# zju3dv/instant-nvr

Measured on AMD Instinct MI355X. Metric: ray-samples/sec, higher is better.
Workload: dtype f32

## Files before the change

include/invr.h:

```cpp
#ifndef INVR_H
#define INVR_H

#include <stddef.h>
#include <stdint.h>

#ifdef __cplusplus
extern "C" {
#endif

#define INVR_NUM_PARTS 5
#define INVR_MAX_LEVELS 16
#define INVR_MAX_LINEAR 4
#define INVR_NUM_JOINTS 24

typedef struct InvrGrid {
    const float* dense;
    const float* hash;
    const float* bounds;
    int32_t n_levels;
    int32_t n_features;
    int32_t start_hash;
    int32_t separate_dense;
    int64_t table_len;
    int32_t res[INVR_MAX_LEVELS];
    float cell[INVR_MAX_LEVELS];
    int64_t dense_off[INVR_MAX_LEVELS];
    int32_t sum;
    int32_t sum_over_features;
    int32_t include_input;
    const float* row_sums;
} InvrGrid;

typedef struct InvrMlp {
    const float* weight[INVR_MAX_LINEAR];
    const float* bias[INVR_MAX_LINEAR];
    int32_t dims[INVR_MAX_LINEAR + 1];
    int32_t n_linear;
} InvrMlp;

typedef struct InvrPart {
    InvrGrid grid;
    InvrMlp occ;
    InvrMlp rgb;
    const float* rgb_latent;
    int32_t latent_dim;
    int32_t num_latent_code;
} InvrPart;

typedef struct InvrModel {
    InvrPart part[INVR_NUM_PARTS];
    InvrGrid deform_grid;
    InvrMlp deform_mlp;
// ... 288 lines not shown
```

instant-nvr_amd/_abi.py:

```python
import ctypes as C
import os

import torch

from . import params
from .config import NUM_PARTS, PART_NAMES

HERE = os.path.dirname(os.path.abspath(__file__))
LIB_PATH = os.environ.get('INVR_LIB_PATH') or os.path.join(HERE, 'libinvr.so')

MAX_LEVELS, MAX_LINEAR, STATS_LEN = 16, 4, 16
_f32p, _f64p, _i32p, _i64p, _u8p = C.POINTER(C.c_float), C.POINTER(C.c_double), C.POINTER(C.c_int32), C.POINTER(C.c_int64), C.POINTER(C.c_uint8)


class InvrGrid(C.Structure):
    _fields_ = [('dense', C.c_void_p), ('hash', C.c_void_p), ('bounds', C.c_void_p),
                ('n_levels', C.c_int32), ('n_features', C.c_int32), ('start_hash', C.c_int32),
                ('separate_dense', C.c_int32), ('table_len', C.c_int64),
                ('res', C.c_int32 * MAX_LEVELS), ('cell', C.c_float * MAX_LEVELS),
                ('dense_off', C.c_int64 * MAX_LEVELS),
                ('sum', C.c_int32), ('sum_over_features', C.c_int32), ('include_input', C.c_int32),
                ('row_sums', C.c_void_p)]


class InvrMlpBwdOut(C.Structure):
    _fields_ = [('g_emb', C.c_void_p), ('gz', C.c_void_p), ('a', C.c_void_p), ('n_pad', C.c_int64), ('g_latent', C.c_void_p)]


class InvrDeformBwdOut(C.Structure):
    _fields_ = [(k, C.c_void_p) for k in ('uvt', 'gfeat', 'gz1', 'gz2', 'gz3', 'a0', 'a1', 'a2')]


class InvrAdamTensor(C.Structure):
    _fields_ = [('param', C.c_void_p), ('grad', C.c_void_p), ('exp_avg', C.c_void_p), ('exp_avg_sq', C.c_void_p),
                ('numel', C.c_int64), ('lr', C.c_float), ('weight_decay', C.c_float), ('bc1', C.c_float), ('bc2_sqrt', C.c_float),
                ('active', C.c_void_p), ('grad_shift', C.c_int32), ('step', C.c_int32)]


class InvrPartGrads(C.Structure):
    _fields_ = [('row_grad', C.c_void_p), ('occ_w', C.c_void_p * 4), ('occ_b', C.c_void_p * 4), ('rgb_w', C.c_void_p * 4),
                ('rgb_b', C.c_void_p * 4), ('rgb_latent', C.c_void_p)]


class InvrTrainGrads(C.Structure):
    _fields_ = [('part', InvrPartGrads * NUM_PARTS), ('deform_dense', C.c_void_p), ('deform_hash', C.c_void_p),
# ... 130 lines not shown
    return {
        'invr_grid_points': (C.c_int, [f3, f3, i3, i64, i64, vp, vp]),
        'invr_mesh_workspace_bytes': (size, [i3]),
        'invr_mesh_workspace_layout': (C.c_int, [i3, C.POINTER(InvrMeshLayout)]),
        'invr_mesh_count': (C.c_int, [vp, i3, f32, vp, size, vp, vp]),
        'invr_mesh_emit': (C.c_int, [vp, i3, f3, f3, f32, vp, size, vp, i64, vp, i64, vp, vp]),
    }


def _signatures_batch():
    i32, vp = C.c_int32, C.c_void_p
    return {
        'invr_patch_batch': (C.c_int, [vp, vp, i32, i32, i32, i32, i32, i32, _f32p, _f64p, _f64p, _f64p, _f32p, vp, vp, vp, vp, vp, vp, vp, vp, vp]),
    }


def _signatures_sample():
    i32, vp = C.c_int32, C.c_void_p
    return {
        'invr_ray_batch': (C.c_int, [vp, vp, vp, vp, i32, i32, vp, i32, _f64p, _f64p, _f64p, _f64p, _f32p, vp, vp, vp, vp, vp, vp, vp]),
    }


SIGNATURES = _signatures()
SIGNATURES_PERCEPTUAL = _signatures_perceptual()
SIGNATURES_MESH = _signatures_mesh()
SIGNATURES_BATCH = _signatures_batch()
SIGNATURES_SAMPLE = _signatures_sample()
EXPORTS = list(SIGNATURES)
ABI_VERSION = 2
BWD_HEAD, BWD_DEFORMER, BWD_ALL = 1, 64, 127
EVAL_RESULT_BYTES = 64
NUM_STAGES = 14
STAGE_NAMES = ['cull', 'knn', 'warp'] + ['encode_%d' % p for p in range(5)] + ['mlp_%d' % p for p in range(5)] + ['composite']

_lib = None


def lib():
    global _lib
    if _lib is None:
        if not os.path.exists(LIB_PATH):
            raise RuntimeError('libinvr.so is not built (%s); run `python -c "import __graft_entry__ as g; g.build()"`. '
                               'There is no CPU fallback for the render path.' % LIB_PATH)
        L = C.CDLL(LIB_PATH)
        for name, (restype, argtypes) in (list(SIGNATURES.items()) + list(SIGNATURES_PERCEPTUAL.items()) + list(SIGNATURES_MESH.items())
                                          + list(SIGNATURES_BATCH.items()) + list(SIGNATURES_SAMPLE.items())):
            fn = getattr(L, name)
            fn.restype, fn.argtypes = restype, list(argtypes)
        if L.invr_version() != ABI_VERSION:
            raise RuntimeError('libinvr.so speaks ABI version %d, this binding %d (include/invr.h INVR_ABI_VERSION): rebuild the library '
                               '(python -m invr.build)' % (L.invr_version(), ABI_VERSION))
        for i, t in enumerate((InvrGrid, InvrMlp, InvrPart, InvrModel, InvrScene, InvrWsLayout, InvrMlpBwdOut, InvrAdamTensor, InvrTrainGrads,
                               InvrDeformBwdOut)):
            if L.invr_sizeof(i) != C.sizeof(t):
                raise RuntimeError('libinvr ABI mismatch: struct %s is %d bytes in the library, %d in the binding'
                                   % (t.__name__, L.invr_sizeof(i), C.sizeof(t)))
        _lib = L
    return _lib


def profile_enable(on):
    lib().invr_profile_enable(int(bool(on)))


def profile_read():
    ms = (C.c_float * NUM_STAGES)()
    n = C.c_int32(0)
    check(lib().invr_profile_read(ms, C.byref(n)))
    return {STAGE_NAMES[i]: float(ms[i]) for i in range(NUM_STAGES)}, int(n.value)
# ... 185 lines not shown
```

instant-nvr_amd/build.py:

```python
import os
import subprocess
import sys
from concurrent.futures import ThreadPoolExecutor

HERE = os.path.dirname(os.path.abspath(__file__))
CSRC = os.path.join(HERE, 'csrc')
OUT = os.path.join(HERE, 'libinvr.so')
SOURCES = ['invr_abi.hip', 'k_cull.hip', 'k_knn.hip', 'k_warp.hip', 'k_encode.hip', 'k_mlp.hip', 'k_composite.hip', 'k_rays.hip', 'k_prep.hip', 'k_optim.hip', 'k_mlp_bwd.hip', 'k_train.hip', 'k_metrics.hip', 'k_perceptual.hip', 'k_mesh.hip', 'k_batch.hip', 'k_sample.hip']
INCLUDE = os.path.join(HERE, '..', 'include')


def headers():
    return ([os.path.join(CSRC, h) for h in sorted(os.listdir(CSRC)) if h.endswith('.h')]
            + [os.path.join(INCLUDE, h) for h in ('invr.h', 'invr_perceptual.h', 'invr_mesh.h', 'invr_batch.h', 'invr_sample.h')])


FLAGS = ['--offload-arch=gfx950', '-O3', '-std=c++17', '-fPIC', '-ffp-contract=off', '-fno-slp-vectorize', '-Wall', '-Wno-unused-function']


def hipcc():
    for c in (os.environ.get('HIPCC'), '/opt/rocm/bin/hipcc', 'hipcc'):
        if c and (os.path.sep not in c or os.path.exists(c)):
            return c
    raise RuntimeError('hipcc not found')


def _stale(target, deps):
    if not os.path.exists(target):
        return True
    t = os.path.getmtime(target)
    return any(os.path.getmtime(d) > t for d in deps)


def build(force=False, verbose=True):
    cc = hipcc()
    objdir = os.path.join(HERE, 'build')
    os.makedirs(objdir, exist_ok=True)
# ... 38 lines not shown
```

instant-nvr_amd/config.py:

```python
import copy

PART_NAMES = ['body', 'leg', 'head', 'larm', 'rarm']
NUM_PARTS = 5
PART_BW_MAP = {
    'body': [14, 13, 9, 6, 3, 0],
    'leg': [1, 2, 4, 5, 7, 8, 10, 11],
    'head': [12, 15],
    'larm': [16, 18, 20, 22],
    'rarm': [17, 19, 21, 23],
}
HASH_PRIMES = (1, 19349663, 83492791)


class Node(dict):

    def __getattr__(self, k):
        try:
            return self[k]
        except KeyError:
            raise AttributeError(k)

    def __setattr__(self, k, v):
        self[k] = v

# ... 25 lines not shown
    'tpose_viewdir': True,
    'use_pair_reg': True,
    'use_reg_distortion': True,
    'random_bg': False,
    'latent_code_dim': 8,
    'geo_feature_dim': 16,
    'num_train_frame': 100,
    'num_latent_code': 100,
    'knn_k': 4,
    'use_knn': True,
    'part_deform': False,
    'use_amp': False,
    'use_batch_bounds': True,
    'bbox_overlap': 0.2,
    'pair_loss_weight': 10.0,
    'reg_dist_weight': 0.1,
    'resd_loss_weight': 0.1,
    'train_fused_loss': True,
    'fused_perceptual': True,
    'train_fused': True,
    'train_hip_mlp': True,
    'voxel_size': [0.005, 0.005, 0.005],
    'eval_row_sums': True,
    'use_lpips': False, 'use_ssim': False, 'use_fourier': False, 'use_tv_image': False, 'vgg19_weights': None,
    'patch_size': 64, 'sample_focus': '',
    'N_rand': 1024, 'body_sample_ratio': 0.5, 'face_sample_ratio': 0.0, 'patch_sampling': False,
    'prune_using_geo': False, 'train_with_coord': False, 'sample_using_mse': False,
    'network': {'occ': {'d_hidden': 64, 'n_layers': 1}},
    'viewdir_embedder': {'kwargs': {'res': 4, 'input_dims': 3}},
    'tpose_deformer': {'embedder': {'kwargs': dict(
        n_levels=8, n_features_per_level=2, log2_hashmap_size=14, base_resolution=4, b=1.38,
        sum=False, sum_over_features=True, separate_dense=True, use_batch_bounds=False,
        include_input=True)}},
    'partnet': {
        'body': _part(20, 16, [[-1, -1.2, -0.34], [0.8, 0.7, 0.5]], 2),
        'leg': _part(20, 2, [[-1, -1.2, -0.34], [0.8, -0.3, 0.5]], 1),
        'head': _part(18, 2, [[-0.3, 0.3, -0.3], [0.3, 0.7, 0.3]], 2),
        'larm': _part(15, 2, [[0.2, 0, -0.2], [0.9, 0.35, 0.2]], 1),
        'rarm': _part(15, 2, [[-0.9, 0, -0.2], [-0.2, 0.35, 0.2]], 1),
    },
}


def make_cfg(**overrides):
    d = copy.deepcopy(DEFAULTS)
    table_log2 = overrides.pop('table_log2', None)
# ... 82 lines not shown
```

instant-nvr_amd/csrc/common.h:

```cpp
#pragma once
#include <hip/hip_runtime.h>
#include <stdint.h>
#include "../../include/invr.h"

#define INVR_WAVE 64
#if defined(__HIP_DEVICE_COMPILE__) && !defined(__gfx950__)
#error "libinvr is written for gfx950 (MI355X) only: build with --offload-arch=gfx950"
#endif
#define HASH_P1 19349663ull
#define HASH_P2 83492791ull

void invr_set_error(const char* fmt, ...);
#define INVR_CHECK(cond, ...)                \
    do {                                     \
        if (!(cond)) {                       \
            invr_set_error(__VA_ARGS__);     \
            return 1;                        \
        }                                    \
    } while (0)
#define INVR_HIP(call)                                                              \
    do {                                                                            \
        hipError_t e_ = (call);                                                     \
        if (e_ != hipSuccess) {                                                     \
            invr_set_error("%s failed: %s", #call, hipGetErrorString(e_));          \
// ... 12 lines not shown

static inline int64_t cdiv(int64_t a, int64_t b) { return (a + b - 1) / b; }
static inline size_t align_up(size_t x, size_t a) { return (x + a - 1) / a * a; }

struct GridDev {
    const float* dense;
    const float* hash;
    const float* bounds;
    int32_t L, F, start_hash, separate_dense;
    int64_t T;
    double inv_T;
    int32_t mod_k, mod32;
    uint32_t mod_c;
    int32_t xdelta;
    int32_t mod1r;
    int32_t mod24;
    int32_t res[INVR_MAX_LEVELS];
    float cell[INVR_MAX_LEVELS];
    float rcell[INVR_MAX_LEVELS];
    int64_t dense_off[INVR_MAX_LEVELS];
    int32_t sum, sum_over_features, include_input;
    const float* row_sums;
    int64_t dense_rows;
};

struct VolDev {
    const float* data;
    const float* bounds;
    int32_t dx, dy, dz, c;
};

struct SceneDev {
    const float* R;
    const float* Th;
    const float* A;
    const float* big_A;
    VolDev pbw;
    VolDev tuv;
    const float* part_pts;
    const float* part_pbw;
    const int64_t* lengths2;
    int32_t M;
    const float* frame_dim;
    const int64_t* latent_index;
    float thresh;
    int32_t tpose_viewdir;
// ... 208 lines not shown
}

int launch_grid_encode_generic(const GridDev& g, const float* xyz, int64_t n, float* out, hipStream_t st);
int launch_grid_encode_bwd_generic(const GridDev& g, const float* xyz, const float* gout, int64_t n, float* g_dense,
                                   float* g_hash, float* g_xyz, hipStream_t st, const int32_t* count = nullptr);
int launch_part_encode_bwd_lists(const GridDev& g, const float* x_soa, const float* gout_soa, float* gx_soa, int64_t stride,
                                 int64_t n_max, const int32_t* count, float* rowgrad, hipStream_t st);
int launch_composite_bwd(const float* raw, const float* g_rgb, const float* g_acc, const float* g_w, int64_t n_rays, int S, float eps,
                         float* g_raw, hipStream_t st);
int launch_sample_volume(const VolDev& v, int c0, int nc, const float* pts, int64_t n, float* out, hipStream_t st);
int launch_knn_blend_dense(const SceneDev& s, const float* pose_pts, int64_t n, float* bw, float* dist, int32_t* nn, float* d2,
                           float* w, hipStream_t st);
int launch_warp_deform_dense(const SceneDev& s, const GridDev& dg, const MlpDev& dm, const float* pose_pts,
                             const float* pose_dirs, const float* bw, const uint8_t* flag, int64_t n,
                             float* tpose, float* tdirs, float* resd, hipStream_t st);
int launch_deform_points(const SceneDev& s, const GridDev& dg, const MlpDev& dm, const float* pts, int64_t n, float* out, hipStream_t st);
int launch_distortion(const float* weights, const float* z, int64_t n_rays, int S, float* out, hipStream_t st);
int launch_generate_rays(const double* kinv, const double* r, const double* t, const double* o, const float* bounds,
                         int H, int W, float* ray_d, float* near, float* far, uint8_t* mask, hipStream_t st);
int launch_adam_advance(void* tensors, int n, double b1, double b2, hipStream_t st);
int launch_adam(const void* tensors, const int32_t* chunk_tensor, const int32_t* chunk_index, int64_t n_chunks, double b1, double b2,
                float eps, hipStream_t st);
int launch_row_sums(const GridDev& g, float* out, hipStream_t st);
int launch_rigid_transformation(const double* poses, const double* joints, const int32_t* parents, float* A, hipStream_t st);
int launch_pack_parts(const float* ppts, const float* weights, const int64_t* parts, const float* tpose, int n_verts, int n_w,
                      int stride, float overlap, float* part_pts, float* part_pbw, int64_t* lengths2, float* bounds, hipStream_t st);
int launch_composite(const float* raw, int64_t n_rays, int S, float eps, float* weights, float* rgb_map, float* acc_map, hipStream_t st);
size_t eval_workspace_bytes(int H, int W);
int launch_image_assemble(const float* pred, const float* gt, const uint8_t* mask, int64_t n, int H, int W, float* img_pred,
                          float* img_gt, uint8_t* u8_pred, uint8_t* u8_gt, void* result, void* ws, hipStream_t st);
int launch_image_metrics(const float* img_pred, const float* img_gt, int H, int W, int crop, void* result, void* ws, hipStream_t st);
```

instant-nvr_amd/csrc/grid_level.h:

```cpp
#pragma once
#include "common.h"

template <int FC = 0>
__device__ __forceinline__ const float* grid_level_table(const GridDev& g, int l, bool hashed) {
    const int F = FC ? FC : g.F;
    return g.separate_dense ? (hashed ? g.hash + (int64_t)(l - g.start_hash) * g.T * F : g.dense + g.dense_off[l] * F)
                            : g.hash + (int64_t)l * g.T * F;
}
template <int FC = 0>
__device__ __forceinline__ const float* grid_level_table(const GridDev& g, int l) { return grid_level_table<FC>(g, l, l >= g.start_hash); }
template <typename T>
__device__ __forceinline__ T* grid_level_like(const GridDev& g, bool hashed, const float* tab, T* dense, T* hash) {
    return g.separate_dense ? (hashed ? hash + (tab - g.hash) : dense + (tab - g.dense)) : hash + (tab - g.hash);
}
__host__ __device__ __forceinline__ int64_t grid_level_rs_off(const GridDev& g, int l, bool hashed) {
    return g.separate_dense ? (hashed ? g.dense_rows + (int64_t)(l - g.start_hash) * g.T : g.dense_off[l]) : (int64_t)l * g.T;
}
__host__ __device__ __forceinline__ int64_t grid_level_rs_off(const GridDev& g, int l) { return grid_level_rs_off(g, l, l >= g.start_hash); }
__host__ __device__ __forceinline__ int64_t grid_level_rows(const GridDev& g, int l) {
    return l >= g.start_hash ? g.T : (int64_t)g.res[l] * g.res[l] * g.res[l];
}
__host__ __device__ __forceinline__ void grid_table_rows(const GridDev& g, int64_t& dense_rows, int64_t& hash_rows) {
    dense_rows = g.separate_dense ? g.dense_rows : 0;
    hash_rows = (int64_t)(g.separate_dense ? g.L - g.start_hash : g.L) * g.T;
}
__host__ __device__ __forceinline__ int grid_out_dim(const GridDev& g) {
    return (g.sum ? (g.sum_over_features ? g.L : g.F) : g.L * g.F) + (g.include_input ? 3 : 0);
}

struct GridRowPair { unsigned r0, r1; };
__device__ __forceinline__ GridRowPair grid_row_zpair(const GridDev& g, bool hashed, int res, int c0z, int c1z, int cx, int cy) {
    GridRowPair r;
    if (hashed) {
        const uint64_t hxy = (uint64_t)(uint32_t)cx ^ ((uint64_t)(uint32_t)cy * HASH_P1);
        r.r0 = grid_hash_mod(hxy ^ ((uint64_t)(uint32_t)c0z * HASH_P2), g);
        r.r1 = grid_hash_mod(hxy ^ ((uint64_t)(uint32_t)c1z * HASH_P2), g);
    } else {
        const unsigned rb = ((unsigned)cx * (unsigned)res + (unsigned)cy) * (unsigned)res;
        r.r0 = rb + (unsigned)c0z;
        r.r1 = rb + (unsigned)c1z;
    }
    return r;
}
__device__ __forceinline__ unsigned grid_row(const GridDev& g, bool hashed, int res, int cx, int cy, int cz) {
    if (hashed) return grid_hash_mod((uint64_t)(uint32_t)cx ^ ((uint64_t)(uint32_t)cy * HASH_P1) ^ ((uint64_t)(uint32_t)cz * HASH_P2), g);
    return ((unsigned)cx * (unsigned)res + (unsigned)cy) * (unsigned)res + (unsigned)cz;
}
// ... 34 lines not shown
```

instant-nvr_amd/csrc/invr_abi.hip:

```cpp
#include <stdarg.h>
#include <stdio.h>
#include <string.h>
#include <math.h>
#include <stdlib.h>
#include <vector>
#include "pipeline.h"
#include "grid_level.h"
#include "train.h"

static thread_local char g_err[512] = "";

void invr_set_error(const char* fmt, ...) {
    va_list ap;
    va_start(ap, fmt);
    vsnprintf(g_err, sizeof(g_err), fmt, ap);
    va_end(ap);
}

extern "C" const char* invr_last_error(void) { return g_err; }
extern "C" int invr_version(void) { return INVR_ABI_VERSION; }
extern "C" size_t invr_sizeof(int32_t which) {
    switch (which) {
        case 0: return sizeof(InvrGrid);
        case 1: return sizeof(InvrMlp);
        case 2: return sizeof(InvrPart);
        case 3: return sizeof(InvrModel);
        case 4: return sizeof(InvrScene);
        case 5: return sizeof(InvrWsLayout);
        case 6: return sizeof(InvrMlpBwdOut);
        case 7: return sizeof(InvrAdamTensor);
        case 8: return sizeof(InvrTrainGrads);
// ... 30 lines not shown
    }
    for (int l = 0; l < INVR_MAX_LEVELS; ++l) {
        d.res[l] = g->res[l]; d.cell[l] = g->cell[l]; d.dense_off[l] = g->dense_off[l];
        d.rcell[l] = 0.0f;
        const float b = g->cell[l];
        uint32_t bits;
        memcpy(&bits, &b, 4);
        if (l < g->n_levels && b > 9.6e-7f && b < 1.0e6f && (bits & 0x7fffffu) != 0x7fffffu) {
            const float y0 = (float)(1.0 / (double)b);
            float best = y0;
            double err = fabs(1.0 - (double)b * (double)y0);
            for (float c : {nextafterf(y0, 0.0f), nextafterf(y0, INFINITY)}) {
                const double e = fabs(1.0 - (double)b * (double)c);
                if (e < err) { err = e; best = c; }
            }
            d.rcell[l] = best;
        }
    }
    d.sum = g->sum; d.sum_over_features = g->sum_over_features; d.include_input = g->include_input;
    d.row_sums = (g->sum && g->sum_over_features) ? g->row_sums : nullptr;
    d.dense_rows = 0;
    if (g->separate_dense)
        for (int l = 0; l < g->start_hash && l < INVR_MAX_LEVELS; ++l) d.dense_rows += (int64_t)g->res[l] * g->res[l] * g->res[l];
    return d;
}

MlpDev make_mlp_dev(const InvrMlp* m) {
    MlpDev d;
    memset(&d, 0, sizeof(d));
    for (int i = 0; i < INVR_MAX_LINEAR; ++i) { d.w[i] = m->weight[i]; d.b[i] = m->bias[i]; }
    for (int i = 0; i <= INVR_MAX_LINEAR; ++i) d.dims[i] = m->dims[i];
    d.n_linear = m->n_linear;
    return d;
}

SceneDev make_scene_dev(const InvrScene* s) {
    SceneDev d;
    memset(&d, 0, sizeof(d));
    d.R = s->R; d.Th = s->Th; d.A = s->A; d.big_A = s->big_A;
    d.pbw = VolDev{s->pbw, s->pbounds, s->pbw_dims[0], s->pbw_dims[1], s->pbw_dims[2], s->pbw_channels};
    d.tuv = VolDev{s->tuv, s->tbounds, s->tuv_dims[0], s->tuv_dims[1], s->tuv_dims[2], 2};
    d.part_pts = s->part_pts; d.part_pbw = s->part_pbw; d.lengths2 = s->lengths2; d.M = s->part_stride;
    d.frame_dim = s->frame_dim; d.latent_index = s->latent_index;
    d.thresh = s->smpl_thresh; d.tpose_viewdir = s->tpose_viewdir; d.comp_eps = s->composite_eps; d.aggr = s->aggr;
    auto g = [](double d) { double w = exp(-d * d / (2.0 * 0.075 * 0.075)); return d * w / (w + 1e-8); };
    const double th = (double)s->smpl_thresh;
    d.near_hi2 = __builtin_inff(); d.band_lo2 = 0.f;
    const double lo = th * 1.01;
    if (th > 0 && lo < 0.42 && g(lo) >= th * 1.002 && g(0.42) >= th * 1.05) {
        double a = 0.42, b = 0.8;
        for (int it = 0; it < 60; ++it) { double m = 0.5 * (a + b); if (g(m) >= th * 1.05) a = m; else b = m; }
        d.near_hi2 = (float)(lo * lo * 1.0001);
        d.band_lo2 = (float)(a * a * 0.9999);
    }
    return d;
}

static int check_grid(const InvrGrid* g, const char* what) {
    INVR_CHECK(g->n_levels >= 1 && g->n_levels <= INVR_MAX_LEVELS, "%s: n_levels %d out of range", what, g->n_levels);
    INVR_CHECK(g->n_features >= 1 && g->n_features <= 16, "%s: n_features %d out of range", what, g->n_features);
    INVR_CHECK(g->hash != nullptr && g->bounds != nullptr, "%s: null table/bounds", what);
    INVR_CHECK(!g->separate_dense || g->dense != nullptr, "%s: separate_dense without dense table", what);
    INVR_CHECK(g->table_len > 1 && g->table_len < (1ll << 31), "%s: table_len out of range", what);
    for (int l = 0; l < g->n_levels; ++l) INVR_CHECK(g->res[l] >= 2 && g->res[l] <= 8192, "%s: level %d resolution %d out of range", what, l, g->res[l]);
    return 0;
}

static int check_mlp_deform(const InvrMlp* m) {
    INVR_CHECK(m->n_linear == 3 && m->dims[0] == 19 && m->dims[1] == 32 && m->dims[2] == 32 && m->dims[3] == 3,
               "deformer MLP must be 19-32-32-3");
    return 0;
}

static int check_deformer(const InvrModel* m) { return check_grid(&m->deform_grid, "deformer grid") || check_mlp_deform(&m->deform_mlp); }

static int check_deformer_slices(const InvrModel* m) {
    if (check_deformer(m)) return 1;
    INVR_CHECK(m->deform_grid.n_levels == 8 && m->deform_grid.n_features == 2 && !m->deform_grid.sum && m->deform_grid.include_input,
               "deformer grid must be 8 levels x 2 features, sum=False, include_input");
    return 0;
}

static RenderArgs scene_args(const InvrScene* scene, int64_t n_rays, int32_t n_samples) {
    RenderArgs a;
    memset(&a, 0, sizeof(a));
    a.scene = make_scene_dev(scene);
    a.R = n_rays; a.S = n_samples; a.N = n_rays * (int64_t)n_samples;
// ... 607 lines not shown
                               int32_t n_verts, int32_t n_weights, int32_t stride, float bbox_overlap,
                               float* part_pts, float* part_pbw, int64_t* lengths2, float* bounds, void* stream) {
    INVR_CHECK(ppts && weights && parts && tpose && part_pts && part_pbw && lengths2 && bounds, "invr_pack_parts: null pointer");
    INVR_CHECK(n_verts >= 0 && n_weights >= 1 && stride >= n_verts, "invr_pack_parts: stride must be >= n_verts");
    return launch_pack_parts(ppts, weights, parts, tpose, n_verts, n_weights, stride, bbox_overlap, part_pts, part_pbw, lengths2,
                             bounds, (hipStream_t)stream);
}

extern "C" int64_t invr_grid_row_sums_len(const InvrGrid* grid) {
    if (!grid || grid->n_levels < 1 || grid->n_levels > INVR_MAX_LEVELS) return 0;
    int64_t drows, hrows;
    grid_table_rows(make_grid_dev(grid), drows, hrows);
    return drows + hrows;
}

extern "C" int invr_grid_row_sums(const InvrGrid* grid, float* out, void* stream) {
    INVR_CHECK(grid && out, "invr_grid_row_sums: null pointer");
    if (check_grid(grid, "grid")) return 1;
    INVR_CHECK(grid->sum && grid->sum_over_features, "invr_grid_row_sums: only sum && sum_over_features grids have row sums");
    INVR_CHECK(grid->n_features % 4 == 0, "invr_grid_row_sums: n_features must be a multiple of 4");
    return launch_row_sums(make_grid_dev(grid), out, (hipStream_t)stream);
}

extern "C" int32_t invr_adam_chunk_elems(void) { return 16384; }

extern "C" int invr_adam_advance(InvrAdamTensor* tensors, int32_t n, double beta1, double beta2, void* stream) {
    INVR_CHECK(n == 0 || tensors, "invr_adam_advance: null pointer");
    return launch_adam_advance(tensors, n, beta1, beta2, (hipStream_t)stream);
}

extern "C" int invr_adam_step(const InvrAdamTensor* tensors, const int32_t* chunk_tensor, const int32_t* chunk_index,
                              int64_t n_chunks, double beta1, double beta2, float eps, void* stream) {
    INVR_CHECK(n_chunks == 0 || (tensors && chunk_tensor && chunk_index), "invr_adam_step: null pointer");
    INVR_CHECK(n_chunks >= 0 && n_chunks < (1ll << 31), "invr_adam_step: bad chunk count");
    return launch_adam(tensors, chunk_tensor, chunk_index, n_chunks, beta1, beta2, eps, (hipStream_t)stream);
}

extern "C" int invr_part_mlp_fwd(const InvrModel* model, int32_t pid, const int64_t* latent_index, const float* emb_soa,
                                 const float* dirs_soa, int64_t n, const int32_t* count_dev, float* raw, void* stream) {
    INVR_CHECK(model && latent_index && pid >= 0 && pid < INVR_NUM_PARTS, "invr_part_mlp_fwd: bad model/pid");
    if (n == 0) return 0;
    INVR_CHECK(emb_soa && dirs_soa && count_dev && raw, "invr_part_mlp_fwd: null pointer");
    PartMlpDev pm = make_part_mlp(model, pid, latent_index);
    return launch_part_mlp(pm, emb_soa, dirs_soa, n, count_dev, n, reinterpret_cast<float4*>(raw), (hipStream_t)stream);
}

// ... 272 lines not shown
```

instant-nvr_amd/csrc/k_encode.hip:

```cpp
#include "pipeline.h"
#include "grid_generic.h"

__global__ void k_grid_encode_rt(GridDev g, const float* xyz, int64_t n, float* out, int out_dim) {
    int64_t i = (int64_t)blockIdx.x * blockDim.x + threadIdx.x;
    if (i >= n) return;
    float x[3];
    grid_normalise(g, xyz + i * 3, x);
    float* o = out + i * out_dim;
    int off = 0;
    if (g.include_input) { o[0] = x[0]; o[1] = x[1]; o[2] = x[2]; off = 3; }
    float tot[16];
    for (int f = 0; f < 16; ++f) tot[f] = 0.0f;
    for (int l = 0; l < g.L; ++l) {
        int64_t rows[8];
        float wts[8];
        const float* tab = grid_level_lookup(g, l, x, rows, wts);
        float acc[16];
        for (int f = 0; f < 16; ++f) acc[f] = 0.0f;
        for (int k = 0; k < 8; ++k)
            for (int f = 0; f < g.F; ++f) acc[f] = fmaf(wts[k], tab[rows[k] * g.F + f], acc[f]);
        if (!g.sum) {
            for (int f = 0; f < g.F; ++f) o[off + l * g.F + f] = acc[f];
        } else if (g.sum_over_features) {
            float s = 0.0f;
// ... 450 lines not shown
}

#define RS_BLOCK 256
#define ENC_LDS_ROWS 4096
__shared__ float g_enc_tab[ENC_LDS_ROWS + 2];
template <bool FASTDIV = false, bool LDSTAB = false>
__device__ __forceinline__ float level_rowsum(const GridDev& g, const float* __restrict__ rs, int hstart, int l, float x, float y, float z) {
    const int res = g.res[l];
    const float cell = g.cell[l];
    int c0x, c1x, c0y, c1y, c0z, c1z;
    float tx, ty, tz;
    const float rcell = g.rcell[l];
    if (FASTDIV) {
        level_corners_fast(x, cell, rcell, res, c0x, c1x, tx);
        level_corners_fast(y, cell, rcell, res, c0y, c1y, ty);
        level_corners_fast(z, cell, rcell, res, c0z, c1z, tz);
    } else {
        level_corners(x, cell, rcell, res, c0x, c1x, tx);
        level_corners(y, cell, rcell, res, c0y, c1y, ty);
        level_corners(z, cell, rcell, res, c0z, c1z, tz);
    }
    unsigned row[8];
    const float* tab;
    if (l >= g.start_hash) {
        tab = rs + g.dense_rows + (int64_t)(l - hstart) * g.T;
        const uint64_t hy0 = (uint64_t)(uint32_t)c0y * HASH_P1, hz0 = (uint64_t)(uint32_t)c0z * HASH_P2;
        const int dy = c1y - c0y, dz = c1z - c0z;
        const uint64_t hx[2] = {(uint64_t)(uint32_t)c0x, (uint64_t)(uint32_t)c1x};
        const uint64_t hy[2] = {hy0, hy0 + (dy > 0 ? HASH_P1 : 0ull) + (dy > 1 ? HASH_P1 : 0ull)};
        const uint64_t hz[2] = {hz0, hz0 + (dz > 0 ? HASH_P2 : 0ull) + (dz > 1 ? HASH_P2 : 0ull)};
        if (g.xdelta) {
            const uint32_t m = (uint32_t)c0x ^ (uint32_t)c1x;
            if (g.mod1r) {
#pragma unroll
                for (int k = 0; k < 4; ++k) {
                    const uint64_t X = hx[0] ^ hy[(k >> 1) & 1] ^ hz[k & 1];
                    const uint32_t r0 = hash_mod24_1r(X, g.mod_k, g.mod_c, (uint32_t)g.T);
                    row[k] = r0;
                    uint32_t r1 = r0 + m - 2u * ((uint32_t)X & m);
                    r1 = min(r1, r1 + (uint32_t)g.T);
                    r1 = min(r1, r1 - (uint32_t)g.T);
                    row[4 + k] = r1;
                }
            } else {
#pragma unroll
                for (int k = 0; k < 4; ++k) {
                    const uint64_t X = hx[0] ^ hy[(k >> 1) & 1] ^ hz[k & 1];
                    const uint32_t r0 = hash_mod24_2r(X, g.mod_k, g.mod_c, (uint32_t)g.T);
                    row[k] = r0;
                    uint32_t r1 = r0 + m - 2u * ((uint32_t)X & m);
                    r1 = min(r1, r1 + (uint32_t)g.T);
                    r1 = min(r1, r1 - (uint32_t)g.T);
                    row[4 + k] = r1;
                }
            }
        } else if (g.mod24) {
#pragma unroll
            for (int k = 0; k < 8; ++k) row[k] = hash_mod24(hx[k >> 2] ^ hy[(k >> 1) & 1] ^ hz[k & 1], g.mod_k, g.mod_c, (uint32_t)g.T);
        } else {
#pragma unroll
            for (int k = 0; k < 8; ++k) row[k] = grid_hash_mod(hx[k >> 2] ^ hy[(k >> 1) & 1] ^ hz[k & 1], g);
        }
    } else {
        tab = g.separate_dense ? rs + g.dense_off[l] : rs + (int64_t)l * g.T;
        const unsigned ures = (unsigned)res;
        const unsigned bx0 = __umul24((unsigned)c0x, ures), bx1 = __umul24((unsigned)c1x, ures);
        const unsigned b00 = __umul24(bx0 + (unsigned)c0y, ures), b01 = __umul24(bx0 + (unsigned)c1y, ures);
        const unsigned b10 = __umul24(bx1 + (unsigned)c0y, ures), b11 = __umul24(bx1 + (unsigned)c1y, ures);
        const unsigned z0 = (unsigned)min(c0z, res - 2);
        const bool s0 = (unsigned)c0z != z0, s1 = (unsigned)c1z != z0;
        const bool far1 = (unsigned)c1z > z0 + 1u;
        const unsigned bb[4] = {b00, b01, b10, b11};
        float vv[8];
        float2 pr[4];
        if (LDSTAB) {
#pragma unroll
            for (int j = 0; j < 4; ++j) pr[j] = make_float2(g_enc_tab[bb[j] + z0], g_enc_tab[bb[j] + z0 + 1u]);
        } else {
#pragma unroll
            for (int j = 0; j < 4; ++j) __builtin_memcpy(&pr[j], tab + bb[j] + z0, sizeof(float2));
        }
#pragma unroll
        for (int j = 0; j < 4; ++j) {
            vv[2 * j] = s0 ? pr[j].y : pr[j].x;
            vv[2 * j + 1] = s1 ? pr[j].y : pr[j].x;
        }
        if (far1) {
// ... 102 lines not shown
            else emb[(int64_t)(3 + la) * a.cap + i] = level_rowsum<false>(g, rs, hstart, la, x, y, z);
            if (fast && g.rcell[lb] != 0.0f) emb[(int64_t)(3 + lb) * a.cap + i] = level_rowsum<true>(g, rs, hstart, lb, x, y, z);
            else emb[(int64_t)(3 + lb) * a.cap + i] = level_rowsum<false>(g, rs, hstart, lb, x, y, z);
        }
    }
}

__global__ void k_row_sums(const float* __restrict__ tab, int64_t rows, int F, float* __restrict__ out) {
    const int per = F / 4;
    const int64_t t = (int64_t)blockIdx.x * blockDim.x + threadIdx.x;
    const int64_t r = t / per;
    if (r >= rows) return;
    const int q = (int)(t - r * per);
    const float4 a = reinterpret_cast<const float4*>(tab)[r * per + q];
    float s = (a.x + a.y) + (a.z + a.w);
    if (per == 4) {
        s = quad_sum(s);
        if (q == 0) out[r] = s;
    } else {
        atomicAdd(out + r, s);
    }
}

int launch_row_sums(const GridDev& g, float* out, hipStream_t st) {
    const int per = g.F / 4;
    auto run = [&](const float* tab, int64_t rows, float* o) -> int {
        if (rows == 0) return 0;
        if (per != 4) INVR_HIP(hipMemsetAsync(o, 0, rows * sizeof(float), st));
        hipLaunchKernelGGL(k_row_sums, dim3((unsigned)cdiv(rows * per, 256)), dim3(256), 0, st, tab, rows, g.F, o);
        INVR_LAUNCH_CHECK();
        return 0;
    };
    int64_t drows, hrows;
    grid_table_rows(g, drows, hrows);
    if (run(g.dense, drows, out)) return 1;
    return run(g.hash, hrows, out + drows);
}

int launch_part_encode_rows_all(const EncodeAllArgs& a, hipStream_t st) {
    for (int p = 0; p < INVR_NUM_PARTS; ++p)
        if (!part_grid_supported(a.g[p], "part encoder kernel", true, false)) return 1;
    int64_t tiles = cdiv(a.cap, 64 * ENC_WAVES);
    unsigned grid = (unsigned)(tiles < 256 * 4 ? (tiles > 0 ? tiles : 1) : 256 * 4);
    hipLaunchKernelGGL(k_part_encode_rows_all, dim3(grid, INVR_NUM_PARTS), dim3(ENC_BLOCK), 0, st, a);
    INVR_LAUNCH_CHECK();
    return 0;
// ... 27 lines not shown
```

instant-nvr_amd/network.py:

```python
import ctypes as C

import numpy as np
import torch
import torch.nn as nn

from . import _abi, params
from .config import cfg as global_cfg, PART_NAMES, NUM_PARTS, validate as validate_cfg


class Embedder(nn.Module):

    def __init__(self, spec, pid=-1, partname='undefined'):
        super().__init__()
        self.spec, self.pid, self.partname = spec, pid, partname
        L, F, T = spec['L'], spec['F'], spec['T']
        ng = dict(requires_grad=False)
        self.bounds = nn.Parameter(torch.from_numpy(spec['bbox'].copy()), **ng)
        self.entries_size = nn.Parameter(torch.from_numpy(spec['size'].copy()), **ng)
        self.entries_num = nn.Parameter(torch.tensor(spec['res'], dtype=torch.int64), **ng)
        self.entries_min = nn.Parameter(torch.zeros(L, dtype=torch.int64), **ng)
        self.entries_cnt = nn.Parameter(torch.tensor(spec['cnt'], dtype=torch.int64), **ng)
        self.entries_sum = nn.Parameter(torch.tensor(spec['cnt'], dtype=torch.int64).cumsum(0), **ng)
        self.start_hash, self.n_levels, self.f, self.out_dim = spec['start_hash'], L, F, spec['out_dim']
        self.n_entries_per_level = T
        self.separate_dense = spec['separate_dense']
        self.use_batch_bounds = spec['use_batch_bounds']
        if self.separate_dense:
            data = torch.zeros((L, T, F))
            nn.init.kaiming_normal_(data)
            self.dense = nn.Parameter(torch.cat([data[i, :spec['cnt'][i]] for i in range(self.start_hash)], 0))
            self.hash = nn.Parameter(data[self.start_hash:].clone())
        else:
            self.hash = nn.Parameter(torch.zeros((L, T, F)))
            nn.init.kaiming_normal_(self.hash)
        self.offsets = nn.Parameter(torch.from_numpy(params.CORNER_OFFSETS.copy()), **ng)

    def __getstate__(self):
        d = self.__dict__.copy()
        for k in ('_rs', '_rs_key', '_row_grad', 'row_grad_dirty'):
            d.pop(k, None)
        return d

    def maybe_adopt_batch_bounds(self, batch):
        if self.use_batch_bounds and 'iter_step' in batch and batch['iter_step'] == 1:
            self.bounds = nn.Parameter(batch['bounds'][0][self.pid].detach().clone(), requires_grad=False)

    def grid_struct(self, keep):
        return _abi.make_grid(self.spec, self.dense if self.separate_dense else None, self.hash, self.bounds, keep)

    def invalidate_row_sums(self):
        self._rs_key = None
        self._rs = None

    def train(self, mode=True):
        self.invalidate_row_sums()
        return super().train(mode)

    def _load_from_state_dict(self, *args, **kwargs):
        self.invalidate_row_sums()
        return super()._load_from_state_dict(*args, **kwargs)

    def row_sums(self):
        tabs = [self.hash] + ([self.dense] if self.separate_dense else [])
        key = tuple((t.data_ptr(), t._version, str(t.device)) for t in tabs)
        if getattr(self, '_rs_key', None) != key:
            keep = []
            g = self.grid_struct(keep)
            n = _abi.lib().invr_grid_row_sums_len(C.byref(g))
            rs = torch.empty(n, device=self.hash.device, dtype=torch.float32)
            _abi.check(_abi.lib().invr_grid_row_sums(C.byref(g), _abi.ptr(rs), _abi.stream_ptr()))
            self._rs, self._rs_key = rs, key
        return self._rs

    def row_grad(self):
        rg = getattr(self, '_row_grad', None)
        if rg is None or rg.device != self.hash.device:
            keep = []
            g = self.grid_struct(keep)
            n = _abi.lib().invr_grid_row_sums_len(C.byref(g))
            rg = torch.zeros(n, device=self.hash.device, dtype=torch.float32)
            self._row_grad = rg
            self.row_grad_dirty = False
        return rg

    def expand_row_grad(self, accumulate=False):
        keep = []
        g = self.grid_struct(keep)
        gh = torch.empty_like(self.hash)
        gd = torch.empty_like(self.dense) if self.separate_dense else None
        _abi.check(_abi.lib().invr_expand_row_grad(C.byref(g), _abi.ptr(self.row_grad()), _abi.ptr(gd), _abi.ptr(gh), _abi.stream_ptr()))
        for p_, g_ in ((self.hash, gh),) + (((self.dense, gd),) if self.separate_dense else ()):
            p_.grad = g_ if (p_.grad is None or not accumulate) else p_.grad + g_
        return gd, gh

    def forward(self, xyz, batch=None):
# ... 93 lines not shown
    def __getstate__(self):
        d = self.__dict__.copy()
        for k in self._TRANSIENT:
            d.pop(k, None)
        return d

    def __setstate__(self, d):
        self.__dict__.update(d)
        self._ws = None

    def model_struct(self, keep):
        params_now = list(self.named_parameters())
        key = tuple(p.data_ptr() for _, p in params_now)
        if getattr(self, '_model_key', None) != key:
            self._model_keep = []
            self._model_base = _abi.make_model(dict(params_now), self.cfg, self._model_keep)
            self._model_key = key
        keep.extend(self._model_keep)
        m = _abi.InvrModel.from_buffer_copy(self._model_base)
        if not self.training and self.cfg.get('eval_row_sums', True):
            for i, pn in enumerate(self.tpose_human.part_networks):
                e = pn.embedder
                if e.spec['sum'] and e.spec['sum_over_features'] and e.f % 4 == 0:
                    rs = e.row_sums()
                    keep.append(rs)
                    m.part[i].grid.row_sums = rs.data_ptr()
        return m

    def workspace(self, nbytes, device):
        if self._ws is None or self._ws.numel() < nbytes or self._ws.device != device:
            self._ws = torch.empty(nbytes, dtype=torch.uint8, device=device)
        self._ws_gen = getattr(self, '_ws_gen', 0) + 1
        return self._ws

    def adopt_batch_bounds(self, batch):
        for pn in self.tpose_human.part_networks:
            pn.embedder.maybe_adopt_batch_bounds(batch)

    def prepare(self, batch):
        self.adopt_batch_bounds(batch)
        keep = []
        return RenderContext(self.model_struct(keep), _abi.make_scene(batch, self.cfg, keep), keep)

    def forward(self, wpts, viewdir, dists, batch):
        L = _abi.lib()
        ctx = batch if isinstance(batch, RenderContext) else self.prepare(batch)
        x = wpts.detach().to(torch.float32).contiguous()
# ... 84 lines not shown
```

instant-nvr_amd/params.py:

```python
from collections import OrderedDict

import numpy as np

from .config import PART_NAMES, NUM_PARTS

CORNER_OFFSETS = np.array([[0, 0, 0], [0, 0, 1], [0, 1, 0], [0, 1, 1],
                           [1, 0, 0], [1, 0, 1], [1, 1, 0], [1, 1, 1]], dtype=np.float32)


def next_prime(n):
    def is_prime(m):
        if m < 2:
            return False
        if m % 2 == 0:
            return m == 2
        i = 3
        while i * i <= m:
            if m % i == 0:
                return False
            i += 2
        return True
    m = n + 1
    while not is_prime(m):
        m += 1
# ... 3 lines not shown
def grid_spec(n_levels=16, n_features_per_level=16, b=1.38, log2_hashmap_size=18, base_resolution=2,
              sum=True, sum_over_features=True, separate_dense=True, use_batch_bounds=True,
              include_input=True, bbox=((0, 0, 0), (1, 1, 1)), **_unused):
    L, F = int(n_levels), int(n_features_per_level)
    T = next_prime(2 ** int(log2_hashmap_size))
    res = [int(base_resolution * b ** i) for i in range(L)]
    cnt = [r ** 3 for r in res]
    size = np.array([1 / (r - 1) for r in res]).astype(np.float32)
    start_hash = L
    for i in range(L):
        if cnt[i] > T:
            start_hash = i
            break
    sep = bool(separate_dense and start_hash)
    csum = np.cumsum(np.array(cnt, dtype=np.int64))
    dense_off = [0] + [int(c) for c in csum[:-1]]
    out_dim = (L if sum_over_features else F) if sum else L * F
    out_dim += 3 if include_input else 0
    return dict(L=L, F=F, T=T, res=res, cnt=cnt, size=size, start_hash=start_hash, separate_dense=sep,
                dense_rows=int(csum[start_hash - 1]) if sep else 0, dense_off=dense_off,
                n_hash=L - start_hash if sep else L, sum=bool(sum), sum_over_features=bool(sum_over_features),
                include_input=bool(include_input), use_batch_bounds=bool(use_batch_bounds),
                bbox=np.asarray(bbox, dtype=np.float32).reshape(2, 3), out_dim=out_dim)


def part_grid_spec(cfg, partname):
    pc = cfg.partnet[partname]
    return grid_spec(bbox=pc.bbox, **pc.embedder.kwargs)


def deformer_grid_spec(cfg):
    return grid_spec(**cfg.tpose_deformer.embedder.kwargs)


def mlp_dims(cfg, partname):
    emb = part_grid_spec(cfg, partname)['out_dim']
    occ = cfg.network.occ
    occ_dims = [emb] + [occ['d_hidden']] * occ['n_layers'] + [1 + cfg.geo_feature_dim]
    vres = cfg.viewdir_embedder.kwargs['res']
    dir_dim = 3 + 3 * 2 * vres
    rgb_in = emb + dir_dim + cfg.geo_feature_dim + cfg.latent_code_dim
    ck = cfg.partnet[partname].color_network.kwargs
    rgb_dims = [rgb_in] + [ck['d_hidden']] * ck['n_layers'] + [3]
    return occ_dims, rgb_dims


# ... 53 lines not shown
```

Baseline: 15.15 billion.

## Precompute per-vertex row-sum tables for hashed levels to skip hashing at eval

For hash levels whose full vertex grid fits within a row limit, the code precomputes a dense per-vertex table of feature sums at eval time and indexes it directly in the encode kernel instead of computing spatial hashes. This removes the hash arithmetic and makes lookups spatially coherent, in exchange for extra device memory and a one-time build whenever the weights change. It also adds an ABI field and new entry points.

New measurement: 15.51 billion (median of 6 runs). 2.4% higher.

```diff
diff --git a/include/invr.h b/include/invr.h
--- a/include/invr.h
+++ b/include/invr.h
@@ -28,6 +28,7 @@
     int32_t sum;
     int32_t sum_over_features;
     int32_t include_input;
+    int32_t vertex_rows;
     const float* row_sums;
 } InvrGrid;
 
diff --git a/include/invr_vertex.h b/include/invr_vertex.h
--- /dev/null
+++ b/include/invr_vertex.h
@@ -0,0 +1,19 @@
+#ifndef INVR_VERTEX_H
+#define INVR_VERTEX_H
+
+#include "invr.h"
+
+#ifdef __cplusplus
+extern "C" {
+#endif
+
+#define INVR_VERTEX_MAX_ROWS 16777216
+
+int64_t invr_grid_vertex_sums_len(const InvrGrid* grid, int64_t max_rows);
+int invr_grid_vertex_sums(const InvrGrid* grid, int64_t max_rows, float* out, void* stream);
+
+#ifdef __cplusplus
+}
+#endif
+
+#endif
diff --git a/instant-nvr_amd/_abi.py b/instant-nvr_amd/_abi.py
--- a/instant-nvr_amd/_abi.py
+++ b/instant-nvr_amd/_abi.py
@@ -20,7 +20,7 @@
                 ('res', C.c_int32 * MAX_LEVELS), ('cell', C.c_float * MAX_LEVELS),
                 ('dense_off', C.c_int64 * MAX_LEVELS),
                 ('sum', C.c_int32), ('sum_over_features', C.c_int32), ('include_input', C.c_int32),
-                ('row_sums', C.c_void_p)]
+                ('vertex_rows', C.c_int32), ('row_sums', C.c_void_p)]
 
 
 class InvrMlpBwdOut(C.Structure):
@@ -197,7 +197,16 @@
     }
 
 
+def _signatures_vertex():
+    i64, vp = C.c_int64, C.c_void_p
+    return {
+        'invr_grid_vertex_sums_len': (i64, [vp, i64]),
+        'invr_grid_vertex_sums': (C.c_int, [vp, i64, vp, vp]),
+    }
+
+
 SIGNATURES = _signatures()
+SIGNATURES_VERTEX = _signatures_vertex()
 SIGNATURES_PERCEPTUAL = _signatures_perceptual()
 SIGNATURES_MESH = _signatures_mesh()
 SIGNATURES_BATCH = _signatures_batch()
@@ -220,7 +229,7 @@
                                'There is no CPU fallback for the render path.' % LIB_PATH)
         L = C.CDLL(LIB_PATH)
         for name, (restype, argtypes) in (list(SIGNATURES.items()) + list(SIGNATURES_PERCEPTUAL.items()) + list(SIGNATURES_MESH.items())
-                                          + list(SIGNATURES_BATCH.items()) + list(SIGNATURES_SAMPLE.items())):
+                                          + list(SIGNATURES_BATCH.items()) + list(SIGNATURES_SAMPLE.items()) + list(SIGNATURES_VERTEX.items())):
             fn = getattr(L, name)
             fn.restype, fn.argtypes = restype, list(argtypes)
         if L.invr_version() != ABI_VERSION:
diff --git a/instant-nvr_amd/build.py b/instant-nvr_amd/build.py
--- a/instant-nvr_amd/build.py
+++ b/instant-nvr_amd/build.py
@@ -12,7 +12,7 @@
 
 def headers():
     return ([os.path.join(CSRC, h) for h in sorted(os.listdir(CSRC)) if h.endswith('.h')]
-            + [os.path.join(INCLUDE, h) for h in ('invr.h', 'invr_perceptual.h', 'invr_mesh.h', 'invr_batch.h', 'invr_sample.h')])
+            + [os.path.join(INCLUDE, h) for h in ('invr.h', 'invr_perceptual.h', 'invr_mesh.h', 'invr_batch.h', 'invr_sample.h', 'invr_vertex.h')])
 
 
 FLAGS = ['--offload-arch=gfx950', '-O3', '-std=c++17', '-fPIC', '-ffp-contract=off', '-fno-slp-vectorize', '-Wall', '-Wno-unused-function']
diff --git a/instant-nvr_amd/config.py b/instant-nvr_amd/config.py
--- a/instant-nvr_amd/config.py
+++ b/instant-nvr_amd/config.py
@@ -71,6 +71,7 @@
     'train_hip_mlp': True,
     'voxel_size': [0.005, 0.005, 0.005],
     'eval_row_sums': True,
+    'eval_vertex_rows': 1 << 24,
     'use_lpips': False, 'use_ssim': False, 'use_fourier': False, 'use_tv_image': False, 'vgg19_weights': None,
     'patch_size': 64, 'sample_focus': '',
     'N_rand': 1024, 'body_sample_ratio': 0.5, 'face_sample_ratio': 0.0, 'patch_sampling': False,
diff --git a/instant-nvr_amd/csrc/common.h b/instant-nvr_amd/csrc/common.h
--- a/instant-nvr_amd/csrc/common.h
+++ b/instant-nvr_amd/csrc/common.h
@@ -58,6 +58,8 @@
     int32_t sum, sum_over_features, include_input;
     const float* row_sums;
     int64_t dense_rows;
+    const float* vertex_sums;
+    int64_t vertex_off[INVR_MAX_LEVELS];
 };
 
 struct VolDev {
@@ -312,6 +314,7 @@
 int launch_adam(const void* tensors, const int32_t* chunk_tensor, const int32_t* chunk_index, int64_t n_chunks, double b1, double b2,
                 float eps, hipStream_t st);
 int launch_row_sums(const GridDev& g, float* out, hipStream_t st);
+int launch_vertex_sums(const GridDev& g, int64_t max_rows, float* out, hipStream_t st);
 int launch_rigid_transformation(const double* poses, const double* joints, const int32_t* parents, float* A, hipStream_t st);
 int launch_pack_parts(const float* ppts, const float* weights, const int64_t* parts, const float* tpose, int n_verts, int n_w,
                       int stride, float overlap, float* part_pts, float* part_pbw, int64_t* lengths2, float* bounds, hipStream_t st);
diff --git a/instant-nvr_amd/csrc/grid_level.h b/instant-nvr_amd/csrc/grid_level.h
--- a/instant-nvr_amd/csrc/grid_level.h
+++ b/instant-nvr_amd/csrc/grid_level.h
@@ -23,6 +23,17 @@
 __host__ __device__ __forceinline__ void grid_table_rows(const GridDev& g, int64_t& dense_rows, int64_t& hash_rows) {
     dense_rows = g.separate_dense ? g.dense_rows : 0;
     hash_rows = (int64_t)(g.separate_dense ? g.L - g.start_hash : g.L) * g.T;
+}
+#define GRID_VERTEX_MAX_ROWS (1ll << 24)
+__host__ __device__ __forceinline__ int64_t grid_vertex_layout(const GridDev& g, int64_t max_rows, int64_t* off) {
+    int64_t total = 0;
+    for (int l = 0; l < INVR_MAX_LEVELS; ++l) {
+        const int64_t rows = (int64_t)g.res[l] * g.res[l] * g.res[l];
+        const bool own = l >= g.start_hash && l < g.L && rows <= max_rows && max_rows <= GRID_VERTEX_MAX_ROWS;
+        off[l] = own ? total : -1;
+        if (own) total += rows;
+    }
+    return total ? total + 2 : 0;
 }
 __host__ __device__ __forceinline__ int grid_out_dim(const GridDev& g) {
     return (g.sum ? (g.sum_over_features ? g.L : g.F) : g.L * g.F) + (g.include_input ? 3 : 0);
diff --git a/instant-nvr_amd/csrc/invr_abi.hip b/instant-nvr_amd/csrc/invr_abi.hip
--- a/instant-nvr_amd/csrc/invr_abi.hip
+++ b/instant-nvr_amd/csrc/invr_abi.hip
@@ -7,6 +7,8 @@
 #include "pipeline.h"
 #include "grid_level.h"
 #include "train.h"
+#include "../../include/invr_vertex.h"
+static_assert(GRID_VERTEX_MAX_ROWS == INVR_VERTEX_MAX_ROWS, "one limit");
 
 static thread_local char g_err[512] = "";
 
@@ -83,6 +85,12 @@
     d.dense_rows = 0;
     if (g->separate_dense)
         for (int l = 0; l < g->start_hash && l < INVR_MAX_LEVELS; ++l) d.dense_rows += (int64_t)g->res[l] * g->res[l] * g->res[l];
+    for (int l = 0; l < INVR_MAX_LEVELS; ++l) d.vertex_off[l] = -1;
+    if (d.row_sums && g->vertex_rows > 0 && g->n_levels >= 1 && g->n_levels <= INVR_MAX_LEVELS) {
+        int64_t drows, hrows;
+        grid_table_rows(d, drows, hrows);
+        if (grid_vertex_layout(d, g->vertex_rows, d.vertex_off) > 0) d.vertex_sums = d.row_sums + drows + hrows;
+    }
     return d;
 }
 
@@ -124,6 +132,7 @@
     INVR_CHECK(!g->separate_dense || g->dense != nullptr, "%s: separate_dense without dense table", what);
     INVR_CHECK(g->table_len > 1 && g->table_len < (1ll << 31), "%s: table_len out of range", what);
     for (int l = 0; l < g->n_levels; ++l) INVR_CHECK(g->res[l] >= 2 && g->res[l] <= 8192, "%s: level %d resolution %d out of range", what, l, g->res[l]);
+    INVR_CHECK(g->vertex_rows >= 0 && g->vertex_rows <= GRID_VERTEX_MAX_ROWS, "%s: vertex_rows %d outside [0, 2^24]", what, g->vertex_rows);
     return 0;
 }
 
@@ -777,6 +786,30 @@
     return launch_row_sums(make_grid_dev(grid), out, (hipStream_t)stream);
 }
 
+extern "C" int64_t invr_grid_vertex_sums_len(const InvrGrid* grid, int64_t max_rows) {
+    if (!grid || grid->n_levels < 1 || grid->n_levels > INVR_MAX_LEVELS || max_rows <= 0) return 0;
+    if (max_rows > GRID_VERTEX_MAX_ROWS) {
+        invr_set_error("invr_grid_vertex_sums_len: max_rows %lld above the limit of 2^24 vertices per level", (long long)max_rows);
+        return -1;
+    }
+    int64_t off[INVR_MAX_LEVELS];
+    return grid_vertex_layout(make_grid_dev(grid), max_rows, off);
+}
+
+extern "C" int invr_grid_vertex_sums(const InvrGrid* grid, int64_t max_rows, float* out, void* stream) {
+    INVR_CHECK(grid, "invr_grid_vertex_sums: null pointer");
+    if (check_grid(grid, "grid")) return 1;
+    INVR_CHECK(max_rows >= 0 && max_rows <= GRID_VERTEX_MAX_ROWS, "invr_grid_vertex_sums: max_rows %lld outside [0, 2^24] vertices per level",
+               (long long)max_rows);
+    INVR_CHECK(grid->sum && grid->sum_over_features && grid->row_sums, "invr_grid_vertex_sums: needs grid->row_sums (invr_grid_row_sums)");
+    GridDev g = make_grid_dev(grid);
+    g.vertex_sums = nullptr;
+    int64_t off[INVR_MAX_LEVELS];
+    if (grid_vertex_layout(g, max_rows, off) == 0) return 0;
+    INVR_CHECK(out, "invr_grid_vertex_sums: null pointer");
+    return launch_vertex_sums(g, max_rows, out, (hipStream_t)stream);
+}
+
 extern "C" int32_t invr_adam_chunk_elems(void) { return 16384; }
 
 extern "C" int invr_adam_advance(InvrAdamTensor* tensors, int32_t n, double beta1, double beta2, void* stream) {
diff --git a/instant-nvr_amd/csrc/k_encode.hip b/instant-nvr_amd/csrc/k_encode.hip
--- a/instant-nvr_amd/csrc/k_encode.hip
+++ b/instant-nvr_amd/csrc/k_encode.hip
@@ -496,7 +496,8 @@
     }
     unsigned row[8];
     const float* tab;
-    if (l >= g.start_hash) {
+    const bool vtab = l >= g.start_hash && g.vertex_sums && g.vertex_off[l] >= 0;
+    if (l >= g.start_hash && !vtab) {
         tab = rs + g.dense_rows + (int64_t)(l - hstart) * g.T;
         const uint64_t hy0 = (uint64_t)(uint32_t)c0y * HASH_P1, hz0 = (uint64_t)(uint32_t)c0z * HASH_P2;
         const int dy = c1y - c0y, dz = c1z - c0z;
@@ -536,7 +537,8 @@
             for (int k = 0; k < 8; ++k) row[k] = grid_hash_mod(hx[k >> 2] ^ hy[(k >> 1) & 1] ^ hz[k & 1], g);
         }
     } else {
-        tab = g.separate_dense ? rs + g.dense_off[l] : rs + (int64_t)l * g.T;
+        tab = vtab ? g.vertex_sums + g.vertex_off[l]
+                   : g.separate_dense ? rs + g.dense_off[l] : rs + (int64_t)l * g.T;
         const unsigned ures = (unsigned)res;
         const unsigned bx0 = __umul24((unsigned)c0x, ures), bx1 = __umul24((unsigned)c1x, ures);
         const unsigned b00 = __umul24(bx0 + (unsigned)c0y, ures), b01 = __umul24(bx0 + (unsigned)c1y, ures);
@@ -685,6 +687,28 @@
     }
 }
 
+__global__ void k_vertex_sums(GridDev g, const float* __restrict__ rs, int l, int64_t rows, float* __restrict__ out) {
+    const int64_t i = (int64_t)blockIdx.x * blockDim.x + threadIdx.x;
+    if (i >= rows) return;
+    const int res = g.res[l];
+    const int cz = (int)(i % res), cy = (int)(i / res % res), cx = (int)(i / ((int64_t)res * res));
+    out[i] = rs[grid_level_rs_off(g, l, true) + grid_row(g, true, res, cx, cy, cz)];
+}
+
+int launch_vertex_sums(const GridDev& g, int64_t max_rows, float* out, hipStream_t st) {
+    int64_t off[INVR_MAX_LEVELS];
+    const int64_t total = grid_vertex_layout(g, max_rows, off);
+    if (total == 0) return 0;
+    for (int l = 0; l < g.L; ++l) {
+        if (off[l] < 0) continue;
+        const int64_t rows = (int64_t)g.res[l] * g.res[l] * g.res[l];
+        hipLaunchKernelGGL(k_vertex_sums, dim3((unsigned)cdiv(rows, 256)), dim3(256), 0, st, g, g.row_sums, l, rows, out + off[l]);
+        INVR_LAUNCH_CHECK();
+    }
+    INVR_HIP(hipMemsetAsync(out + total - 2, 0, 2 * sizeof(float), st));
+    return 0;
+}
+
 int launch_row_sums(const GridDev& g, float* out, hipStream_t st) {
     const int per = g.F / 4;
     auto run = [&](const float* tab, int64_t rows, float* o) -> int {
diff --git a/instant-nvr_amd/network.py b/instant-nvr_amd/network.py
--- a/instant-nvr_amd/network.py
+++ b/instant-nvr_amd/network.py
@@ -37,7 +37,7 @@
 
     def __getstate__(self):
         d = self.__dict__.copy()
-        for k in ('_rs', '_rs_key', '_row_grad', 'row_grad_dirty'):
+        for k in ('_rs', '_rs_key', '_vs', '_vs_key', '_row_grad', 'row_grad_dirty'):
             d.pop(k, None)
         return d
 
@@ -51,6 +51,8 @@
     def invalidate_row_sums(self):
         self._rs_key = None
         self._rs = None
+        self._vs_key = None
+        self._vs = None
 
     def train(self, mode=True):
         self.invalidate_row_sums()
@@ -71,6 +73,28 @@
             _abi.check(_abi.lib().invr_grid_row_sums(C.byref(g), _abi.ptr(rs), _abi.stream_ptr()))
             self._rs, self._rs_key = rs, key
         return self._rs
+
+    def vertex_sums(self, max_rows):
+        L = _abi.lib()
+        tabs = [self.hash] + ([self.dense] if self.separate_dense else [])
+        key = tuple((t.data_ptr(), t._version, str(t.device)) for t in tabs) + (int(max_rows),)
+        if getattr(self, '_vs_key', None) != key:
+            n_vs = params.vertex_layout(self.spec, max_rows)[1]
+            buf = None
+            if n_vs:
+                keep = []
+                g = self.grid_struct(keep)
+                n_rs = L.invr_grid_row_sums_len(C.byref(g))
+                assert L.invr_grid_vertex_sums_len(C.byref(g), int(max_rows)) == n_vs, (self.partname, n_vs)
+                buf = torch.empty(n_rs + n_vs, device=self.hash.device, dtype=torch.float32)
+                _abi.check(L.invr_grid_row_sums(C.byref(g), _abi.ptr(buf), _abi.stream_ptr()))
+                g.row_sums = buf.data_ptr()
+                _abi.check(L.invr_grid_vertex_sums(C.byref(g), int(max_rows), C.c_void_p(buf.data_ptr() + 4 * n_rs), _abi.stream_ptr()))
+            self._vs, self._vs_key = buf, key
+        return self._vs
+
+    def derived_bytes(self):
+        return sum(t.numel() * t.element_size() for t in (getattr(self, '_rs', None), getattr(self, '_vs', None)) if t is not None)
 
     def row_grad(self):
         rg = getattr(self, '_row_grad', None)
@@ -210,7 +234,11 @@
             for i, pn in enumerate(self.tpose_human.part_networks):
                 e = pn.embedder
                 if e.spec['sum'] and e.spec['sum_over_features'] and e.f % 4 == 0:
-                    rs = e.row_sums()
+                    vrows = int(self.cfg.get('eval_vertex_rows', 0) or 0)
+                    rs = e.vertex_sums(vrows) if vrows > 0 else None
+                    m.part[i].grid.vertex_rows = vrows if rs is not None else 0
+                    if rs is None:
+                        rs = e.row_sums()
                     keep.append(rs)
                     m.part[i].grid.row_sums = rs.data_ptr()
         return m
diff --git a/instant-nvr_amd/params.py b/instant-nvr_amd/params.py
--- a/instant-nvr_amd/params.py
+++ b/instant-nvr_amd/params.py
@@ -49,6 +49,20 @@
                 n_hash=L - start_hash if sep else L, sum=bool(sum), sum_over_features=bool(sum_over_features),
                 include_input=bool(include_input), use_batch_bounds=bool(use_batch_bounds),
                 bbox=np.asarray(bbox, dtype=np.float32).reshape(2, 3), out_dim=out_dim)
+
+
+VERTEX_MAX_ROWS = 2 ** 24
+
+
+def vertex_layout(spec, max_rows):
+    if int(max_rows) > VERTEX_MAX_ROWS:
+        raise ValueError('invr: eval_vertex_rows = %d is above the limit of 2^24 vertices per level' % int(max_rows))
+    off, total = [], 0
+    for l in range(spec['L']):
+        own = l >= spec['start_hash'] and spec['cnt'][l] <= int(max_rows)
+        off.append(total if own else -1)
+        total += spec['cnt'][l] if own else 0
+    return off, (total + 2 if total else 0)
 
 
 def part_grid_spec(cfg, partname):
```
